# kazuto1011/dusty-gan

Measured on AMD Instinct MI355X. Metric: G+D train images/sec on 64x1024 LiDAR (steps/sec beside it), higher is better.
Workload: dtype bf16

## Files before the change

### dusty_gan_amd/_lib.py

```python
import ctypes as C
import os
import subprocess

_HERE = os.path.dirname(os.path.abspath(__file__))
CSRC = os.path.join(_HERE, "csrc")
LIB_PATH = os.path.join(CSRC, "libdustygan_hip.so")
if os.environ.get("DUSTY_GAN_LIB_DIAG"):
    _d = os.environ["DUSTY_GAN_LIB_DIAG"]
    LIB_PATH = os.path.join(CSRC, "libdustygan_hip_diag%s.so" % ("" if _d == "1" else _d))

DG_OK, DG_EINVAL, DG_EUNSUPPORTED, DG_EHIP = 0, 1, 2, 3
DG_F32, DG_BF16 = 0, 1
DG_BF16X2 = 2
MODE_S2, MODE_UP, MODE_GEMM = 0, 1, 2
EPI_LINEAR, EPI_LRELU, EPI_MASK = 0, 1, 2
DG_FORCE_AUTO, DG_FORCE_DIRECT, DG_FORCE_MFMA, DG_FORCE_THIN, DG_FORCE_LOCKSTEP, DG_FORCE_PINGPONG = 0, 1, 2, 3, 4, 5
DG_FORCE_WG_REGSTAGED, DG_FORCE_WG_DMA_PAIRS, DG_FORCE_WG_DMA_NOPAIRS, DG_FORCE_PINGPONG_SINGLE, DG_FORCE_PROJ_STREAM = 6, 7, 8, 9, 10
DG_FORCE_FP32X3 = 0x100
DG_CONV_FAMILY_DIRECT, DG_CONV_FAMILY_MFMA, DG_CONV_FAMILY_THIN, DG_CONV_FAMILY_LOCKSTEP, DG_CONV_FAMILY_PINGPONG = 1, 2, 3, 4, 5
DG_CONV_FAMILY_PROJ_STREAM = 6
DG_WGRAD_VARIANT_DIRECT, DG_WGRAD_VARIANT_MFMA, DG_WGRAD_VARIANT_THIN, DG_WGRAD_VARIANT_DMA, DG_WGRAD_VARIANT_THIN_MFMA = 1, 2, 3, 5, 7
POLICY_BITS = {"brightness": 1, "saturation": 2, "contrast": 4, "translation": 8, "cutout": 16}

_ERR = {1: "DG_EINVAL (bad argument)", 2: "DG_EUNSUPPORTED (shape not supported by the requested kernel)",
# ... 41 lines not shown
                ("eps", C.c_float), ("ilo", C.c_int), ("ihi", C.c_int), ("n", C.c_long), ("out", C.c_void_p),
                ("out_bf16", C.c_void_p), ("B", C.c_int), ("H", C.c_int), ("W", C.c_int), ("uf", C.c_void_p),
                ("qi", C.c_void_p)]


class DgWgrad(C.Structure):
    _fields_ = [
        ("wmode", C.c_int), ("ring", C.c_int),
        ("B", C.c_int), ("Hc", C.c_int), ("Wc", C.c_int),
        ("Ci", C.c_int), ("Co", C.c_int),
        ("a", C.c_void_p), ("a_sb", C.c_long), ("a_sp", C.c_long), ("a_sc", C.c_long),
        ("g", C.c_void_p), ("g_sb", C.c_long), ("g_sp", C.c_long), ("g_sc", C.c_long),
        ("dw", C.c_void_p), ("scale", C.c_float), ("rowscale", C.c_void_p),
        ("a_dtype", C.c_int), ("g_dtype", C.c_int),
        ("ws", C.c_void_p), ("g_mod", C.c_int),
    ]


XSUM_PARTS = 8


class DgFetch(C.Structure):
    _fields_ = [("pol", C.c_void_p), ("mask", C.c_void_p), ("pool_ctr", C.c_void_p), ("npool", C.c_int),
                ("min_depth", C.c_float), ("max_depth", C.c_float), ("drop_const", C.c_float), ("B", C.c_int), ("HW", C.c_long),
                ("out", C.c_void_p), ("parts", C.c_void_p), ("nslab", C.c_long), ("flip_tab", C.c_void_p)]


class DgAugSet(C.Structure):
    _fields_ = [("x", C.c_void_p), ("xsum", C.c_void_p), ("xsum_parts", C.c_int), ("u_b", C.c_void_p), ("u_c", C.c_void_p), ("t_h", C.c_void_p),
                ("t_w", C.c_void_p), ("o_x", C.c_void_p), ("o_y", C.c_void_p)]


class DgOptSeg(C.Structure):
    _fields_ = [("off", C.c_longlong), ("numel", C.c_longlong), ("part", C.c_void_p), ("splits", C.c_int), ("accumulate", C.c_int),
                ("kind", C.c_int), ("ci", C.c_int), ("co", C.c_int), ("shadow_t", C.c_void_p), ("ws_src", C.c_void_p),
                ("ws_coef", C.c_void_p), ("ws_stride", C.c_longlong), ("ws_n", C.c_int), ("ws_bf16", C.c_int),
                ("ws_scale", C.c_float), ("first_block", C.c_int)]


OPT_MAX_SEG = 20


class DgWgradPlan(C.Structure):
    _fields_ = [("variant", C.c_int), ("splits", C.c_int), ("ws_floats", C.c_long), ("tap_pairs", C.c_int)]


class DgWgradReduce(C.Structure):
    _fields_ = [("ws", C.c_void_p), ("dw", C.c_void_p), ("numel", C.c_long), ("splits", C.c_int), ("accumulate", C.c_int)]


class DgConvPlan(C.Structure):
    _fields_ = [("family", C.c_int), ("bm", C.c_int), ("bn", C.c_int), ("tiles", C.c_int), ("workgroups", C.c_int),
                ("tiles_per_wg", C.c_int), ("thin_mfma", C.c_int), ("mask_bits", C.c_int), ("dbias_rows", C.c_int),
                ("sum_parts", C.c_int)]


_P, _I, _L, _F, _D, _U64 = C.c_void_p, C.c_int, C.c_long, C.c_float, C.c_double, C.c_uint64

PROTOTYPES = {
    "dg_conv": [C.POINTER(DgConv), _I, _P],
    "dg_conv_ex": [C.POINTER(DgConv), _I, _I, _P],
    "dg_conv_plan": [C.POINTER(DgConv), _I, _I, C.POINTER(DgConvPlan)],
    "dg_conv_mfma_supported": [C.POINTER(DgConv)],
    "dg_wgrad": [C.POINTER(DgWgrad), _I, _I, _P],
    "dg_wgrad_plan": [C.POINTER(DgWgrad), _I, _I, C.POINTER(DgWgradPlan)],
    "dg_wgrad_group": [C.POINTER(DgWgrad), _I, _I, _I, _P],
    "dg_wgrad_group_plan": [C.POINTER(DgWgrad), _I, _I, _I, C.POINTER(DgWgradPlan)],
    "dg_wgrad_reduce": [C.POINTER(DgWgradReduce), _I, _P],
    "dg_wgrad_mfma_supported": [C.POINTER(DgWgrad)],
    "dg_wgrad_kernel_variant": [C.POINTER(DgWgrad), _I],
    "dg_wgrad_has_sample_map": [C.POINTER(DgWgrad), _I],
    "dg_blur_fwd": [_P, _P, _I, _I, _I, _I, _I, _P],
    "dg_blur_fwd_mean": [_P, _P, _I, _I, _I, _I, _I, _P, _I, _P, _P],
    "dg_blur_bwd": [_P, _I, _P, _I, _I, _I, _I, _P],
    "dg_blur_bwd_r1": [_P, _I, _P, _F, _P, _I, _I, _I, _I, _P],
    "dg_blur_r1_tangent": [_P, _I, _P, _F, _P, _P, _I, _I, _I, _I, _I, _P],
    "dg_final_fwd": [_P, _I, _P, _P, _F, _I, _L, _P, _P],
    "dg_final_fwd_acc": [_P, _I, _P, _P, _F, _I, _L, _P, _P],
    "dg_final_bwd_data": [_P, _I, _P, _P, _P, _F, _I, _L, _I, _P, _P, _P],
    "dg_batch_wsum": [_P, _I, _P, _F, _I, _L, _P, _P],
    "dg_head_post_fwd": [_P, _P, _P, _I, _I, _F, _F, _I, _L, _P, _P, _P],
    "dg_head_post_fwd_sum": [_P, _P, _P, _I, _I, _F, _F, _I, _L, _P, _P, _P, _P],
    "dg_head_post_bwd": [_P, _P, _P, _P, _P, _I, _F, _F, _I, _L, _F, _F, _P, _P, _P, _I, _P, _P],
    "dg_logistic_noise": [_P, _P, _F, _L, _P, _P],
    "dg_diffaug_fwd": [_P, _P, _P, _P, _P, _P, _P, _I, _I, _I, _I, _P, _P, _P],
    "dg_diffaug_bwd": [_P, _P, _P, _P, _P, _P, _P, _I, _I, _I, _I, _P, _P, _P],
    "dg_diffaug_fwd_acc": [_P, _P, _P, _P, _P, _P, _P, _I, _I, _I, _I, _P, _P, _P],
    "dg_diffaug_fwd_pre": [_P, _P, _P, _P, _P, _P, _P, _I, _I, _I, _I, _P, _P, _P],
    "dg_diffaug_bwd_acc": [_P, _P, _P, _P, _P, _P, _P, _I, _I, _I, _I, _P, _P, _P],
    "dg_diffaug_blur_fwd": [C.POINTER(DgAugSet), _I, _I, _I, _I, _I, _I, _P, _I, _P],
    "dg_blur_bwd_augsum": [_P, _I, _P, _P, _P, _P, _I, _P, _I, _I, _I, _I, _P],
    "dg_diffaug_bwd_pre": [_P, _P, _P, _P, _P, _P, _P, _I, _I, _I, _I, _P, _P, _P],
    "dg_head_post_bwd_aug": [_P, _P, _P, _P, _P, _P, _P, _P, _P, _P, _P, _I, _P, _I, _F, _F, _I, _I, _I, _F, _F, _P, _P, _P,
                             _I, _P, _P],
    "dg_fetch_reals_pool_sum": [_P, _P, _P, _I, _F, _F, _F, _I, _L, _P, _P, _P],
    "dg_fetch_reals_resident_sum": [_P, _P, _L, _P, _F, _F, _F, _I, _L, _P, _P, _P],
    "dg_resident_gather": [_P, _L, _I, _L, _L, _P, _P, _P, _P],
    "dg_nsgan_d": [_P, _P, _I, _F, _P, _P, _P, _P],
    "dg_nsgan_g": [_P, _I, _F, _P, _P, _P],
    "dg_nsgan_d_step": [_P, _P, _I, _F, _P, _P, _P, _P, _P, _P],
    "dg_nsgan_g_step": [_P, _I, _F, _P, _P, _P],
    "dg_gan_d_step": [_I, _F, _P, _P, _I, _F, _P, _P, _P, _P, _P, _P],
    "dg_gan_g_step": [_I, _P, _P, _I, _F, _P, _P, _P],
    "dg_final_gan_bwd": [_I, _I, _F, _P, _P, _I, _F, _I, _P, _P, _P, _P, _P, _P, _I, _P, _F, _L, _I, _P, _P, _P, _P, _P],
    "dg_det_arena": [_P, _L, _P],
    "dg_mean_acc": [_P, _I, _P, _P],
    "dg_fetch_reals": [_P, _P, _F, _F, _F, _L, _P, _P],
    "dg_fetch_reals_sum": [_P, _P, _F, _F, _F, _I, _L, _P, _P, _P],
    "dg_pl_penalty": [_P, _I, _I, _F, _P, _P, _P, _P],
    "dg_head_post_bwd2": [_P, _P, _P, _P, _P, _P, _I, _F, _F, _I, _L, _F, _F, _P, _P, _P, _I, _P],
    "dg_scan_to_polar": [_P, _I, _I, _I, _I, _I, _I, _P, _D, _D, _F, _P, _P, _P, _P, _P],
    "dg_inv_to_xyz": [_P, _P, _I, _I, _I, _I, _F, _F, _F, _F, _P, _P, _P],
    "dg_unit_map": [_P, _L, _I, _P, _P],
    "dg_normals": [_P, _I, _I, _I, _I, _P, _P],
    "dg_scan_project": [_P, _P, _I, _I, _I, _P, _P, _P, _P, _P],
# ... 328 lines not shown
```

### dusty_gan_amd/csrc/conv_mfma_persist_impl.h

```cpp
#pragma once
#include "mfma_common.h"

namespace persist {

template <typename T> struct StageWrite;
template <> struct StageWrite<bf16> {
  static __device__ __forceinline__ void put(unsigned addr, float v) {
    const bf16 h = (bf16)v;
    const unsigned bits = (unsigned)__builtin_bit_cast(unsigned short, h);
    asm volatile("ds_write_b16 %0, %1" ::"v"(addr), "v"(bits) : "memory");
  }
};
template <> struct StageWrite<float> {
  static __device__ __forceinline__ void put(unsigned addr, float v) {
    asm volatile("ds_write_b32 %0, %1" ::"v"(addr), "v"(v) : "memory");
  }
};

struct Tile {
  int nt, xt, px, Y, bt;
};

template <int MODE>
__device__ __forceinline__ bool next_tile(Tile& t, int tiles_n, int tiles_x, int rows) {
  if (++t.nt < tiles_n) return false;
  t.nt = 0;
  if (++t.xt < tiles_x) return false;
  t.xt = 0;
  if (MODE == MODE_UP) {
    if (++t.px < 2) return false;
    t.px = 0;
  }
  if (++t.Y == rows) { t.Y = 0; ++t.bt; }
  return true;
}

template <int MODE>
__host__ __device__ __forceinline__ int pack_htaps(int adj, int Y, int Hc, unsigned long long& list) {
  list = 0;
  int n = 0;
#pragma unroll
  for (int i = 0; i < 6; ++i) {
    int r, ky;
    if (dg_tap1d(MODE, adj, 0, Y, Hc, i, r, ky)) {
      list |= (unsigned long long)((r << 2) | ky) << (10 * n);
      ++n;
    }
  }
  return n;
}

#define DG_WAITV(n) asm volatile("s_waitcnt vmcnt(%0)" ::"n"(n) : "memory")

struct Geo {
  int tiles_n, tiles_x, ntiles;
  int SW, NSB, lsw;
  int dbg;
};

template <typename T, int BM, int BN, int WM, int WN, int SB, int NS, int MODE>
__global__ __launch_bounds__(64 * WM * WN, 1) void conv_kernel(ConvP p, Geo g) {
  constexpr int NWV = WM * WN;
  constexpr int ES = sizeof(T);
  constexpr int BK = SB / ES;
  constexpr int EPC = 16 / ES;
  constexpr int TM = BM / WM / 32, TN = BN / WN / 32;
  constexpr int RPI = 1024 / SB;
  constexpr int CPR = SB / 16;
  constexpr int KS = SB / 32;
  constexpr int STAGE = (BM + BN) * SB;
  constexpr int IA = BM / RPI / NWV, IB = BN / RPI / NWV;
  constexpr int IPT = IA + IB;
  constexpr int E = NS - 1;
  constexpr int WC = BN / WN;
  constexpr int RB = WC * ES;
  constexpr int RS = RB + 16;
  constexpr int CR = RB / 16;
  constexpr int NDB0 = 512;
  constexpr int DBR = sizeof(T) == 4 ? WM : 1;
  constexpr int SR = (NS * STAGE + NWV * 16 * RS + NDB0 * 4 * DBR > 160 * 1024) ? 8 : 16;
  constexpr int CPL = SR * CR / 64;
  constexpr int STRIP = SR * RS;
  constexpr int NQ = 32 / SR;
  constexpr int NST = TM * NQ * CPL;
  constexpr int nW = MODE == MODE_S2 ? 4 : 2;
  static_assert(IA >= 1 && IB >= 1, "piece distribution");
  static_assert(NS >= 3 && NS <= 4 && KS >= 2 && KS % 2 == 0 && 2 * IPT + NST <= 63, "ring / vmcnt immediates");
  constexpr int NDB = 512;
  static_assert(NS * STAGE + NWV * STRIP + NDB * 4 * DBR <= 160 * 1024, "LDS");
  __shared__ __attribute__((aligned(1024))) unsigned char lds[NS * STAGE + NWV * STRIP + NDB * 4 * DBR];

  const int G = gridDim.x;
  const int q8 = G >> 3, r8 = G & 7, xcd = blockIdx.x & 7;
  const int gi = (xcd < r8 ? xcd * (q8 + 1) : r8 * (q8 + 1) + (xcd - r8) * q8) + (blockIdx.x >> 3);
  const int tq = g.ntiles / G, tr = g.ntiles % G;
  const int t0 = gi * tq + (gi < tr ? gi : tr);
  const int tcount = tq + (gi < tr ? 1 : 0);
  if (tcount == 0) return;

  const int tid = threadIdx.x;
  const int KC = p.K / BK;
  const int Ws = MODE == MODE_S2 ? 2 * p.Wc : p.Wc, cmul = MODE == MODE_S2 ? 2 : 1;
  const int Wo = MODE == MODE_S2 ? p.Wc : 2 * p.Wc;
  const int rows = MODE == MODE_S2 ? p.Hc : 2 * p.Hc;
  const int tiles_n = g.tiles_n, tiles_x = g.tiles_x;

  Tile first;
  {
    int mt = t0 / tiles_n;
    first.nt = t0 % tiles_n;
// ... 386 lines not shown
```

### dusty_gan_amd/csrc/conv_mfma_pp.hip

```cpp
#include "conv_mfma_persist_impl.h"

#include <type_traits>

namespace pp {

using persist::Geo;
using persist::Tile;

typedef __attribute__((ext_vector_type(4))) float f32x4_t;

#define PP_WAIT(vm) asm volatile("s_waitcnt vmcnt(%0) lgkmcnt(0)" ::"n"(vm) : "memory")

constexpr int NHT = 256;
struct HTab { unsigned long long e[NHT]; };

__device__ __forceinline__ unsigned long long pp_stamp() {
  unsigned long long t;
  __builtin_amdgcn_sched_barrier(0);
  asm volatile("s_memtime %0\n\ts_waitcnt lgkmcnt(0)" : "=s"(t)::"memory");
  __builtin_amdgcn_sched_barrier(0);
  return t;
}

template <int CTRL>
__device__ __forceinline__ float row_add(float v) {
  const int s = __builtin_amdgcn_update_dpp(0, __builtin_bit_cast(int, v), CTRL, 0xf, 0xf, false);
  return v + __builtin_bit_cast(float, s);
}

template <int BN, int MODE, bool MASK, bool DUAL = false, bool BITS = false, bool X2 = false>
__global__ __launch_bounds__(512, 2) void conv_pp_kernel(ConvP p, Geo g, HTab ht) {
  static_assert(MASK || !BITS, "BITS: a flavour of the EPI_MASK epilogue");
  static_assert(!X2 || !BITS, "X2: mask source = the saved activation's hi half");
  static_assert(!DUAL || (MODE == MODE_UP && BN == 128), "DUAL: both column parities of a 64-channel MODE_UP layer");
  constexpr int NCH = DUAL ? BN / 2 : BN;
  constexpr int BM = 256, NWV = 8, WN = 2;
  constexpr int SB = 128;
  constexpr int WC = BN / WN;
  constexpr int TM = 4, TN = WC / 16;
  constexpr int CPL = 4 * TN;
  constexpr int IMG_ROWS = 264;
  constexpr int AIMG = IMG_ROWS * SB;
  constexpr int BT = BN * SB;
  constexpr int PSTAGE = AIMG + 2 * BT;
  constexpr int NPS = 2;
  constexpr int IA = 4, IB = BN / 8 / NWV;
  constexpr int NST = TM * CPL * 2 / 16;
  constexpr int NDB = 512;
  constexpr int NPAIR = MODE == MODE_S2 ? 2 : 1;
  constexpr bool STRIP = BN == 128 && !X2;
  constexpr int SCR = STRIP ? 16 * WC * 2 : 0;
  constexpr int NDBR = 4;
  constexpr int NDBX = MASK ? (NDBR - 2) * NDB : 0;
  constexpr int DBW = DUAL ? NWV : NWV / WN;
  constexpr int LDS_HT = NPS * PSTAGE + 3 * NDB * 4 + NDBX * 4 + NWV * SCR;
  static_assert(IB >= 1 && LDS_HT <= 160 * 1024, "LDS");
  __shared__ __attribute__((aligned(1024))) unsigned char lds[LDS_HT];
#ifdef DG_PP_DIAG
  constexpr int dbg = DG_PP_DIAG;
#else
  constexpr int dbg = 0;
#endif

  const int G = gridDim.x;
  const int q8 = G >> 3, r8 = G & 7, xcd = blockIdx.x & 7;
  const int gi0 = xcd < r8 ? xcd * (q8 + 1) : r8 * (q8 + 1) + (xcd - r8) * q8;
  const int nwx = q8 + (xcd < r8 ? 1 : 0);
  const int tq = g.ntiles / G, tr = g.ntiles % G;
  const int xs = gi0 * tq + (gi0 < tr ? gi0 : tr);
  const int xe = (gi0 + nwx) * tq + (gi0 + nwx < tr ? gi0 + nwx : tr);
  const int t0 = xs + (int)(blockIdx.x >> 3);
  const int tcount = t0 < xe ? (xe - t0 + nwx - 1) / nwx : 0;
  if (tcount == 0) {
    if (MASK && p.dbias && p.dbias_part)
      for (int n = threadIdx.x; n < p.N; n += 64 * NWV) p.dbias_part[(long)blockIdx.x * p.N + n] = 0.f;
    return;
  }

  const unsigned long long tk0 = (dbg & 8) ? pp_stamp() : 0ull;
  const unsigned long long tr0 = (dbg & 8) ? __builtin_amdgcn_s_memrealtime() : 0ull;
  const int tid = threadIdx.x;
  const int wave = __builtin_amdgcn_readfirstlane(tid >> 6), lane = tid & 63;
  const int KC = p.K / 64;
  const int Ws = MODE == MODE_S2 ? 2 * p.Wc : p.Wc, cmul = MODE == MODE_S2 ? 2 : 1;
  const int Wo = MODE == MODE_S2 ? p.Wc : 2 * p.Wc;
  const int rows = MODE == MODE_S2 ? p.Hc : 2 * p.Hc;
  const int tiles_n = g.tiles_n, tiles_x = g.tiles_x;

  auto tile_at = [&](int t) {
    Tile r;
    int mt = t / tiles_n;
    r.nt = t % tiles_n;
    r.px = 0;
    r.xt = mt % tiles_x; mt /= tiles_x;
    if (MODE == MODE_UP && !DUAL) { r.px = mt & 1; mt >>= 1; }
    r.Y = mt % rows; r.bt = mt / rows;
    r.nt = __builtin_amdgcn_readfirstlane(r.nt); r.xt = __builtin_amdgcn_readfirstlane(r.xt);
    r.px = __builtin_amdgcn_readfirstlane(r.px); r.Y = __builtin_amdgcn_readfirstlane(r.Y);
    r.bt = __builtin_amdgcn_readfirstlane(r.bt);
    return r;
  };
  const Tile first = tile_at(t0);
  Tile dstep;
  {
    int r = nwx;
    dstep.nt = r % tiles_n; r /= tiles_n;
    dstep.xt = r % tiles_x; r /= tiles_x;
    dstep.px = 0;
    if (MODE == MODE_UP && !DUAL) { dstep.px = r & 1; r >>= 1; }
    dstep.Y = r % rows; dstep.bt = r / rows;
    dstep.nt = __builtin_amdgcn_readfirstlane(dstep.nt); dstep.xt = __builtin_amdgcn_readfirstlane(dstep.xt);
    dstep.px = __builtin_amdgcn_readfirstlane(dstep.px); dstep.Y = __builtin_amdgcn_readfirstlane(dstep.Y);
    dstep.bt = __builtin_amdgcn_readfirstlane(dstep.bt);
  }
  auto tile_next = [&](Tile& t) __attribute__((always_inline)) {
    int c;
    t.nt += dstep.nt; c = t.nt >= tiles_n; if (c) t.nt -= tiles_n;
    t.xt += dstep.xt + c; c = t.xt >= tiles_x; if (c) t.xt -= tiles_x;
    if (MODE == MODE_UP && !DUAL) { t.px += dstep.px + c; c = t.px >> 1; t.px &= 1; }
    t.Y += dstep.Y + c; c = t.Y >= rows; if (c) t.Y -= rows;
    t.bt += dstep.bt + c;
  };

  const bf16* in = (const bf16*)p.in;
  const bf16* w = (const bf16*)p.w;
  const int lrow = lane >> 3, pos = lane & 7;
  auto swzA = [](int row) { return ((row >> 1) & 3) << 1; };
  auto swzB = [](int row) { return ((row >> 1) & 1) | (((row / CPL) & 3) << 1); };

  unsigned voffA[NPAIR][IA + 1], voffB[IB];
  int colA[IA + 1];
  unsigned sampA[IA + 1];
  {
    const int pitch = g.SW + (DUAL ? 2 : 1);
#pragma unroll
    for (int u = 0; u <= IA; ++u) {
      const int m = (u < IA ? (wave + NWV * u) : 32) * 8 + lrow;
      int seg = m / pitch, c = m - seg * pitch;
      if (seg >= g.NSB) { seg = 0; c = 0; }
      colA[u] = cmul * c;
      sampA[u] = (unsigned)(seg * (int)p.in_sb * 2 + (pos ^ swzA(m)) * 16);
    }
  }
#pragma unroll
  for (int u = 0; u < IB; ++u) {
    const int row = (wave + NWV * u) * 8 + lrow;
    voffB[u] = (unsigned)((DUAL ? row & 63 : row) * (int)p.w_sn * 2 + (pos ^ swzB(row)) * 16);
  }
  const unsigned dst_wave = (unsigned)wave * 1024u;

  const int wm = wave >> 1, wn = wave & 1;
  const int a16 = lane & 15, g4 = lane >> 4;
  const unsigned lds0 = (unsigned)(size_t)(__attribute__((address_space(3))) unsigned char*)lds;
  unsigned pbase[2];
  {
    const int rowbase = ((wm * 64) >> g.lsw) * (g.SW + (DUAL ? 2 : 1)) + ((wm * 64) & (g.SW - 1));
#pragma unroll
    for (int t = 0; t < 2; ++t) {
      const int r = rowbase + a16 + t + (DUAL ? wn : 0);
      pbase[t] = (unsigned)(r * SB + ((g4 ^ swzA(r)) << 4));
    }
  }
  const unsigned wrow = (unsigned)(wn * WC + (a16 >> 2) * CPL + (a16 & 3));
  const unsigned wbase = (unsigned)(AIMG + wrow * SB + ((g4 ^ (((a16 >> 1) & 1) | ((a16 >> 2) << 1))) << 4));

  float* s_rs = (float*)(lds + NPS * PSTAGE);
  float* s_bias = s_rs + NDB;
  float* s_db = s_bias + NDB;
  const unsigned srs0 = lds0 + NPS * PSTAGE, sbias0 = srs0 + NDB * 4, sdb0 = sbias0 + NDB * 4;
  const bool want_db = MASK && p.dbias != nullptr;
  const bool db_rows = MASK && DBW * p.N <= NDBR * NDB;
  const unsigned sdbw0 = db_rows ? sbias0 + (unsigned)((DUAL ? wave : wave / WN) * p.N) * 4u : sdb0;
  for (int i = tid; i < NDB; i += 64 * NWV) {
    s_bias[i] = (!MASK && p.bias && i < p.N) ? p.bias[i % p.bias_mod] * (p.epi == EPI_LRELU ? SQRT2 : 1.f) : 0.f;
    s_db[i] = 0.f;
// ... 281 lines not shown
      else if (t == 0) { if (wave == 0) PP_WAIT(IA + IB + 1); else PP_WAIT(IA + IB); }
      else PP_WAIT(IB);
      auto finish_tile = [&]() __attribute__((always_inline)) {
        if (!(dbg & 4)) epilogue(tprev);
        else {
#pragma unroll
          for (int i = 0; i < TM; ++i)
#pragma unroll
            for (int jj = 0; jj < TN; ++jj) asm volatile("" ::"v"(acc[i][jj]));
          zero_acc();
        }
        pending = false;
      };
      if (t == 0 && pending && wave >= 4) finish_tile();
      if (stamps) t2 = pp_stamp();
      __builtin_amdgcn_s_barrier();
      if (stamps) t3 = pp_stamp();
      __builtin_amdgcn_sched_barrier(0);
      if (t == 0 && pending) finish_tile();
      __builtin_amdgcn_sched_barrier(0);
      if (comp) {
        if (stamps && tkf == 0) tkf = t3;
#pragma unroll
        for (int ks = 0; ks < 2; ++ks) {
          if (!(dbg & 2)) {
#pragma unroll
            for (int i = 0; i < TM; ++i)
#pragma unroll
              for (int jj = 0; jj < TN; ++jj)
                acc[i][jj] = __builtin_amdgcn_mfma_f32_16x16x32_bf16(__builtin_bit_cast(bf16x8, fw[ks][jj]),
                                                                      __builtin_bit_cast(bf16x8, fp[ks][i]), acc[i][jj], 0, 0, 0);
          }
          if (ks == 0) {
            __builtin_amdgcn_sched_barrier(0);
            if (MASK && last && !(dbg & (4 | 64))) load_aux(tprev);
          }
        }
        if (last) pending = true;
      }
      __builtin_amdgcn_sched_barrier(0);
      if (stamps) t4 = pp_stamp();
      if (ISS || t == 0 || wave < 4) __builtin_amdgcn_s_barrier();
      if (stamps) {
        t5 = pp_stamp();
        tsum[0] += t1 - t0; tsum[1] += t2 - t1; tsum[2] += t3 - t2; tsum[3] += t4 - t3; tsum[4] += t5 - t4;
        tend = t5;
      }
    };
    step(std::integral_constant<int, 0>{});
    step(std::integral_constant<int, 1>{});
    const unsigned sw_ = so_c; so_c = so_i; so_i = sw_;
  };

  Tile ti = first;
  for (int c = 0; c < tcount; ++c) {
    unsigned long long hl;
    int nh;
    {
      const unsigned long long e = ht.e[ti.Y];
      nh = (int)(e >> 60) & 7;
      hl = e & 0x0fffffffffffffffull;
    }
    const char* in_t = (const char*)(in + (long)(ti.bt * g.NSB) * p.in_sb);
    const char* w_t = (const char*)(w + (long)(ti.nt * NCH) * p.w_sn);
    const int x0 = cmul * ti.xt * BM;
#pragma unroll
    for (int pi = 0; pi < NPAIR; ++pi) {
      const int cb = MODE == MODE_S2 ? pi - 1 : ((DUAL || ti.px == 0) ? -1 : 0);
#pragma unroll
      for (int u = 0; u <= IA; ++u)
        voffA[pi][u] = __umul24((unsigned)((x0 + colA[u] + cb) & (Ws - 1)), spb) + sampA[u];
    }
    const int kxa = MODE == MODE_S2 ? 0 : (ti.px == 0 ? 3 : 2), kxb = MODE == MODE_S2 ? 2 : (ti.px == 0 ? 1 : 0);
    bool firstg = true;
    for (int h = 0; h < nh; ++h) {
      const int it_r = (int)(hl & 1023) >> 2, it_ky = (int)hl & 3;
      hl >>= 10;
      const char* sA_row = in_t + (long)it_r * Ws * spb;
      const char* sB_row = w_t + (long)(it_ky * 4) * tap_b;
      for (int kc = 0; kc < (X2 ? 3 : 1) * KC; ++kc) {
        const int kq = X2 ? kc / 3 : kc, sub = X2 ? kc - 3 * kq : 0;
        const char* sA_k = sA_row + kq * (X2 ? 2 * SB : SB) + (sub == 1 ? SB : 0);
        const char* sB_k = sB_row + kq * (X2 ? 2 * SB : SB) + (sub == 2 ? SB : 0);
#pragma unroll
        for (int pi = 0; pi < NPAIR; ++pi) {
          pair_iter(std::true_type{}, firstg, pi, sA_k, sB_k + (long)(kxa + pi) * tap_b, sB_k + (long)(kxb + pi) * tap_b,
                    sB_k + 2 * tap_b, sB_k);
          if (firstg) { firstg = false; warm = false; }
        }
      }
    }
    tprev = ti;
    tile_next(ti);
  }
  pair_iter(std::false_type{}, true, 0, nullptr, nullptr, nullptr, nullptr, nullptr);
  const unsigned long long tk2 = (dbg & 8) ? pp_stamp() : 0ull;
  const unsigned long long tr2 = (dbg & 8) ? __builtin_amdgcn_s_memrealtime() : 0ull;
  if (pending && !(dbg & 4)) {
    asm volatile("s_waitcnt vmcnt(0)" ::: "memory");
    epilogue(tprev);
  }
  if (stamps && blockIdx.x == 0 && lane == 0) {
    float* sink = (float*)p.out + wave * 8;
    asm volatile("s_waitcnt vmcnt(0)" ::: "memory");
    const unsigned long long tk3 = pp_stamp();
    for (int k = 0; k < 6; ++k) sink[k] = (float)tsum[k];
    float* ph = (float*)p.out + 64 + wave * 8;
    ph[0] = (float)(tk1 - tk0); ph[1] = (float)(tkf - tk0); ph[2] = (float)(tk2 - tk0); ph[3] = (float)(tk3 - tk0);
    ph[4] = (float)tcount;
    ph[5] = (float)(tr2 - tr0);
  }
  if (want_db) {
    asm volatile("s_waitcnt vmcnt(0) lgkmcnt(0)" ::: "memory");
    __syncthreads();
    for (int n = tid; n < p.N; n += 64 * NWV) {
      float v;
      if (db_rows) {
        v = s_bias[n];
#pragma unroll
        for (int r = 1; r < DBW; ++r) v += s_bias[r * p.N + n];
      } else v = s_db[n];
      if (p.dbias_part) p.dbias_part[(long)blockIdx.x * p.N + n] = v;
      else atomicAdd(&p.dbias[n % p.bias_mod], v);
    }
  }
}

template <int BN, int MODE, bool MASK, bool DUAL = false, bool X2 = false>
int launch(const ConvP* p, const Geo& g0, hipStream_t stream, int wg_cap, DgConvPlan* plan) {
  constexpr int CPL_ = (BN / 2 / 16) * 4;
  const bool bits_ok = !X2 && p->out_sn == 1 && p->out_sb % 8 == 0 && p->out_sp % CPL_ == 0 && p->N % CPL_ == 0;
  if (!MASK && p->mask_out && !bits_ok) return DG_EUNSUPPORTED;
  const bool bits = MASK && p->mask_in && bits_ok;
  Geo g = g0;
  static int resident = 0;
  if (!resident) {
    int dev = 0, cus = 0;
    HIP_CHECK_RET(hipGetDevice(&dev));
    HIP_CHECK_RET(hipDeviceGetAttribute(&cus, hipDeviceAttributeMultiprocessorCount, dev));
    resident = cus;
  }
  g.dbg = 0;
  const int cap = (wg_cap > 0 && wg_cap < resident) ? wg_cap : resident;
  const int G = g.ntiles < cap ? g.ntiles : cap;
  if (plan) {
    plan->family = DG_CONV_FAMILY_PINGPONG; plan->bm = DUAL ? 512 : 256; plan->bn = DUAL ? BN / 2 : BN; plan->tiles = g.ntiles; plan->workgroups = G;
    plan->tiles_per_wg = (g.ntiles + G - 1) / G;
    plan->mask_bits = MASK ? (bits ? 2 : 0) : 1;
    plan->dbias_rows = (MASK && (DUAL ? 8 : 4) * p->N <= 2048) ? G : 0;
    return DG_OK;
  }
  HTab ht;
  {
    const int rows = MODE == MODE_S2 ? p->Hc : 2 * p->Hc;
    for (int y = 0; y < NHT; ++y) {
      unsigned long long hl = 0;
      const int nh = y < rows ? persist::pack_htaps<MODE>(p->adj, y, p->Hc, hl) : 0;
      ht.e[y] = hl | ((unsigned long long)nh << 60);
    }
  }
  if constexpr (X2) {
    conv_pp_kernel<BN, MODE, MASK, DUAL, false, true><<<(unsigned)G, 512, 0, stream>>>(*p, g, ht);
  } else if constexpr (MASK) {
    if (bits) conv_pp_kernel<BN, MODE, true, DUAL, true><<<(unsigned)G, 512, 0, stream>>>(*p, g, ht);
    else conv_pp_kernel<BN, MODE, true, DUAL, false><<<(unsigned)G, 512, 0, stream>>>(*p, g, ht);
  } else conv_pp_kernel<BN, MODE, false, DUAL><<<(unsigned)G, 512, 0, stream>>>(*p, g, ht);
  HIP_CHECK_RET(hipGetLastError());
  return DG_OK;
}

}

int dg_conv_mfma_pp_launch(const ConvP* p0, hipStream_t stream, int min_tiles, int wg_cap, DgConvPlan* plan, int dual) {
  if (p0->mode != MODE_S2 && p0->mode != MODE_UP) return DG_EUNSUPPORTED;
  const bool x2 = p0->in_dtype == DG_BF16X2;
  if (p0->in_dtype != p0->out_dtype || p0->in_dtype != p0->w_dtype || (p0->in_dtype != DG_BF16 && !x2)) return DG_EUNSUPPORTED;
  ConvP q = *p0;
  if (x2) {
    if (p0->K % 64 || p0->N % 64 || p0->in_sp % 64 || p0->in_sb % 64 || p0->out_sp % 64 || p0->out_sb % 64 || p0->w_sn % 64 ||
        p0->w_st % 64 || (((size_t)p0->in | (size_t)p0->out | (size_t)p0->w | (size_t)p0->aux) & 255))
      return DG_EUNSUPPORTED;
    if (p0->mask_out || p0->mask_in) return DG_EUNSUPPORTED;
    q.in_sb *= 2; q.in_sp *= 2; q.out_sb *= 2; q.out_sp *= 2; q.w_st *= 2; q.w_sn *= 2;
  }
  const ConvP* p = &q;
  if (p->K % 64 != 0 || !p->ring || p->nscale) return DG_EUNSUPPORTED;
  if (p->mode == MODE_UP && p->adj && p->K < 128) return DG_EUNSUPPORTED;
  if (p->in_sk != 1 || p->w_sk != 1 || p->out_sn != 1) return DG_EUNSUPPORTED;
  if (p->out_sp % 8 != 0 || p->in_sp % 8 != 0 || p->w_sn % 8 != 0) return DG_EUNSUPPORTED;
  if (p->N > 512 || (p->bias && p->bias_mod < p->N && p->N % p->bias_mod != 0)) return DG_EUNSUPPORTED;
  if (p->dbias && p->bias_mod < p->N) return DG_EUNSUPPORTED;
  const int Ws = p->mode == MODE_S2 ? 2 * p->Wc : p->Wc;
  if ((Ws & (Ws - 1)) != 0 || p->in_sp * 2 >= (1 << 24)) return DG_EUNSUPPORTED;
  if ((p->mode == MODE_S2 ? p->Hc : 2 * p->Hc) > 256) return DG_EUNSUPPORTED;
  const bool mask = p->epi == EPI_MASK;
  if (mask ? p->bias != nullptr : p->dbias != nullptr) return DG_EUNSUPPORTED;
  if (p->rowscale && p->B > 512) return DG_EUNSUPPORTED;
  persist::Geo g;
  int bn = 0;
  if (dual && p->mode == MODE_UP && p->N % 128 != 0 && p->N % 64 == 0 && persist::make_geo<256, 64>(p, g) && g.SW >= 64 &&
      g.NSB * (g.SW + 2) <= 264 && g.ntiles / 2 >= min_tiles) {
    g.ntiles /= 2;
    if (x2) return mask ? pp::launch<128, MODE_UP, true, true, true>(p, g, stream, wg_cap, plan)
                        : pp::launch<128, MODE_UP, false, true, true>(p, g, stream, wg_cap, plan);
    return mask ? pp::launch<128, MODE_UP, true, true>(p, g, stream, wg_cap, plan)
                : pp::launch<128, MODE_UP, false, true>(p, g, stream, wg_cap, plan);
  }
  if (p->N % 128 == 0 && persist::make_geo<256, 128>(p, g) && g.SW >= 64 && g.ntiles >= min_tiles) bn = 128;
  else if (p->N % 64 == 0 && persist::make_geo<256, 64>(p, g) && g.SW >= 64 && g.ntiles >= min_tiles) bn = 64;
  if (!bn) return DG_EUNSUPPORTED;
  const int sel = (bn == 128 ? 0 : 4) + (p->mode == MODE_UP ? 2 : 0) + (mask ? 1 : 0);
  if (x2) switch (sel) {
    case 0: return pp::launch<128, MODE_S2, false, false, true>(p, g, stream, wg_cap, plan);
    case 1: return pp::launch<128, MODE_S2, true, false, true>(p, g, stream, wg_cap, plan);
    case 2: return pp::launch<128, MODE_UP, false, false, true>(p, g, stream, wg_cap, plan);
    case 3: return pp::launch<128, MODE_UP, true, false, true>(p, g, stream, wg_cap, plan);
    case 4: return pp::launch<64, MODE_S2, false, false, true>(p, g, stream, wg_cap, plan);
    case 5: return pp::launch<64, MODE_S2, true, false, true>(p, g, stream, wg_cap, plan);
    case 6: return pp::launch<64, MODE_UP, false, false, true>(p, g, stream, wg_cap, plan);
    default: return pp::launch<64, MODE_UP, true, false, true>(p, g, stream, wg_cap, plan);
  }
  switch (sel) {
    case 0: return pp::launch<128, MODE_S2, false>(p, g, stream, wg_cap, plan);
// ... 10 lines not shown
```

### include/dusty_gan_hip.h

```cpp
#ifndef DUSTY_GAN_HIP_H
#define DUSTY_GAN_HIP_H
#include <stdint.h>

#ifdef __cplusplus
extern "C" {
#endif

#define DG_OK 0
#define DG_EINVAL 1
#define DG_EUNSUPPORTED 2
#define DG_EHIP 3

#define DG_F32 0
#define DG_BF16 1
#define DG_BF16X2 2

#define DG_MODE_S2 0
#define DG_MODE_UP 1
#define DG_MODE_GEMM 2

#define DG_EPI_LINEAR 0
#define DG_EPI_LRELU 1
#define DG_EPI_MASK 2

// ... 22 lines not shown
  void* mask_out;
  const void* mask_in;
  float* tanh_sum_parts;
} DgConv;
#define DG_UP_FRAG_BYTES (3 * 18 * 1024)
#define DG_DBIAS_SLOTS 32
#define DG_DBIAS_SLOT_FLOATS 1024

typedef struct DgWgrad {
  int wmode, ring;
  int B, Hc, Wc;
  int Ci, Co;
  const void* a;
  long a_sb, a_sp, a_sc;
  const void* g;
  long g_sb, g_sp, g_sc;
  float* dw;
  float scale;
  const float* rowscale;
  int a_dtype, g_dtype;
  float* ws;
  int g_mod;
} DgWgrad;

int dg_conv(const DgConv* p, int force, void* stream);
#define DG_FORCE_AUTO 0
#define DG_FORCE_DIRECT 1
#define DG_FORCE_MFMA 2
#define DG_FORCE_THIN 3
#define DG_FORCE_LOCKSTEP 4
#define DG_FORCE_PINGPONG 5
#define DG_FORCE_WG_REGSTAGED 6
#define DG_FORCE_WG_DMA_PAIRS 7
#define DG_FORCE_WG_DMA_NOPAIRS 8
#define DG_FORCE_PINGPONG_SINGLE 9
#define DG_FORCE_PROJ_STREAM 10
#define DG_FORCE_FP32X3 0x100
#define DG_CONV_FAMILY_DIRECT 1
#define DG_CONV_FAMILY_MFMA 2
#define DG_CONV_FAMILY_THIN 3
#define DG_CONV_FAMILY_LOCKSTEP 4
#define DG_CONV_FAMILY_PINGPONG 5
#define DG_CONV_FAMILY_PROJ_STREAM 6
typedef struct DgConvPlan {
  int family;
  int bm, bn;
  int tiles;
  int workgroups;
  int tiles_per_wg;
  int thin_mfma;
  int mask_bits;
  int dbias_rows;
  int sum_parts;
} DgConvPlan;
int dg_conv_ex(const DgConv* p, int force, int wg_cap, void* stream);
int dg_conv_plan(const DgConv* p, int force, int wg_cap, DgConvPlan* plan);
int dg_conv_mfma_supported(const DgConv* p);

int dg_wgrad(const DgWgrad* p, int accumulate, int force, void* stream);
#define DG_WGRAD_VARIANT_DIRECT 1
#define DG_WGRAD_VARIANT_MFMA 2
#define DG_WGRAD_VARIANT_THIN 3
#define DG_WGRAD_VARIANT_DMA 5
#define DG_WGRAD_VARIANT_THIN_MFMA 7
typedef struct DgWgradPlan {
  int variant;
  int splits;
  long ws_floats;
  int tap_pairs;
} DgWgradPlan;
int dg_wgrad_plan(const DgWgrad* p, int accumulate, int force, DgWgradPlan* plan);
int dg_wgrad_group(const DgWgrad* items, int n, int force, int rounds, void* stream);
int dg_wgrad_group_plan(const DgWgrad* items, int n, int force, int rounds, DgWgradPlan* plans);
typedef struct DgWgradReduce {
  const float* ws;
  float* dw;
  long numel;
  int splits;
  int accumulate;
} DgWgradReduce;
int dg_wgrad_reduce(const DgWgradReduce* items, int n, void* stream);
int dg_wgrad_mfma_supported(const DgWgrad* p);
int dg_wgrad_kernel_variant(const DgWgrad* p, int force);
int dg_wgrad_has_sample_map(const DgWgrad* p, int force);

int dg_blur_fwd(const float* x, void* out, int dtype, int B, int H, int W, int ring, void* stream);
int dg_blur_fwd_mean(const float* x, void* out, int dtype, int B, int H, int W, int ring, const float* mean_src, int mean_n,
                     float* mean_acc, void* stream);
int dg_blur_bwd(const void* d, int dtype, float* dx, int B, int H, int W, int ring, void* stream);
int dg_blur_bwd_r1(const void* d, int dtype, float* dx, float oscale, float* ssq, int B, int H, int W, int ring, void* stream);
int dg_blur_r1_tangent(const void* d, int dtype, void* out, float oscale, float* ssq, float* mean_acc, int mean_n, int B, int H,
                       int W, int ring, void* stream);

int dg_final_fwd(const void* d4, int dtype, const float* wf, const float* bias, float scale, int B, long n, float* y,
                 void* stream);
int dg_final_fwd_acc(const void* d4, int dtype, const float* wf, const float* bias, float scale, int B, long n, float* y,
                 void* stream);
int dg_final_bwd_data(const void* d4, int dtype, const float* wf, const float* up, const float* rowscale, float scale,
                      int B, long n, int C, void* dd4, float* dbias, void* stream);
int dg_batch_wsum(const void* src, int dtype, const float* coef, float scale, int B, long n, float* out, void* stream);

int dg_head_post_fwd(float* gout, const float* noise_pixel, const float* noise_image, int arch, int training,
                     float tau, float drop_const, int B, long HW, float* mask, float* depth, void* stream);
int dg_head_post_fwd_sum(float* gout, const float* noise_pixel, const float* noise_image, int arch, int training,
                         float tau, float drop_const, int B, long HW, float* mask, float* depth, float* dsum, void* stream);
int dg_head_post_bwd(const float* gout, const float* noise_pixel, const float* noise_image, const float* mask,
                     const float* ddepth, int arch, float tau, float drop_const, int B, long HW, float s_depth,
                     float s_conf, float* draw, float* dbias, void* draw_pm , int cp,
                     float* bias_ws, void* stream);
// ... 209 lines not shown
```

Before: 14020.

## Rotate ping-pong conv tile walk to balance per-workgroup tap load

Replaces the fixed strided tile walk in the persistent ping-pong conv kernel with a parameterised walk. Each workgroup's stride can advance by one extra row of tiles per step, which spreads rows with different vertical-tap counts more evenly across workgroups. The host simulates per-workgroup tap work for both walks and picks the rotated one only when it lowers the maximum. The choice is cached per shape, and the old walk is kept for masked dbias kernels or when an env var requests it. It adds host-side simulation cost on cache misses and a slightly more complex device-side tile increment.

```diff
diff --git a/dusty_gan_amd/_lib.py b/dusty_gan_amd/_lib.py
--- a/dusty_gan_amd/_lib.py
+++ b/dusty_gan_amd/_lib.py
@@ -117,7 +117,10 @@
 class DgConvPlan(C.Structure):
     _fields_ = [("family", C.c_int), ("bm", C.c_int), ("bn", C.c_int), ("tiles", C.c_int), ("workgroups", C.c_int),
                 ("tiles_per_wg", C.c_int), ("thin_mfma", C.c_int), ("mask_bits", C.c_int), ("dbias_rows", C.c_int),
-                ("sum_parts", C.c_int)]
+                ("sum_parts", C.c_int),
+                ("tiles_n", C.c_int), ("tiles_x", C.c_int), ("tile_par", C.c_int), ("tile_rows", C.c_int),
+                ("walk_shift", C.c_int), ("walk_units", C.c_long), ("walk_max_units", C.c_int),
+                ("walk_max_units_old", C.c_int)]
 
 
 _P, _I, _L, _F, _D, _U64 = C.c_void_p, C.c_int, C.c_long, C.c_float, C.c_double, C.c_uint64
@@ -126,6 +129,7 @@
     "dg_conv": [C.POINTER(DgConv), _I, _P],
     "dg_conv_ex": [C.POINTER(DgConv), _I, _I, _P],
     "dg_conv_plan": [C.POINTER(DgConv), _I, _I, C.POINTER(DgConvPlan)],
+    "dg_conv_walk_order": [C.POINTER(DgConvPlan), _I, C.POINTER(C.c_int), _L],
     "dg_conv_mfma_supported": [C.POINTER(DgConv)],
     "dg_wgrad": [C.POINTER(DgWgrad), _I, _I, _P],
     "dg_wgrad_plan": [C.POINTER(DgWgrad), _I, _I, C.POINTER(DgWgradPlan)],
diff --git a/dusty_gan_amd/csrc/conv_mfma_persist_impl.h b/dusty_gan_amd/csrc/conv_mfma_persist_impl.h
--- a/dusty_gan_amd/csrc/conv_mfma_persist_impl.h
+++ b/dusty_gan_amd/csrc/conv_mfma_persist_impl.h
@@ -56,6 +56,7 @@
   int tiles_n, tiles_x, ntiles;
   int SW, NSB, lsw;
   int dbg;
+  int shift = 0;
 };
 
 template <typename T, int BM, int BN, int WM, int WN, int SB, int NS, int MODE>
diff --git a/dusty_gan_amd/csrc/conv_mfma_pp.hip b/dusty_gan_amd/csrc/conv_mfma_pp.hip
--- a/dusty_gan_amd/csrc/conv_mfma_pp.hip
+++ b/dusty_gan_amd/csrc/conv_mfma_pp.hip
@@ -1,5 +1,7 @@
 #include "conv_mfma_persist_impl.h"
 
+#include <cstdlib>
+#include <cstring>
 #include <type_traits>
 
 namespace pp {
@@ -8,6 +10,62 @@
 using persist::Tile;
 
 typedef __attribute__((ext_vector_type(4))) float f32x4_t;
+
+__host__ __device__ __forceinline__ int walk_uni(int v) {
+#if defined(__HIP_DEVICE_COMPILE__)
+  return __builtin_amdgcn_readfirstlane(v);
+#else
+  return v;
+#endif
+}
+
+template <bool PAR>
+struct Walk {
+  Tile t;
+  int count;
+  Tile dn, dw;
+  int pos, nwx, shift, tiles_n, tiles_x, rows;
+
+  __host__ __device__ __forceinline__ Tile digits(int r) const {
+    Tile d;
+    d.nt = r % tiles_n; r /= tiles_n;
+    d.xt = r % tiles_x; r /= tiles_x;
+    d.px = 0;
+    if (PAR) { d.px = r & 1; r >>= 1; }
+    d.Y = r % rows; d.bt = r / rows;
+    d.nt = walk_uni(d.nt); d.xt = walk_uni(d.xt); d.px = walk_uni(d.px); d.Y = walk_uni(d.Y); d.bt = walk_uni(d.bt);
+    return d;
+  }
+  __host__ __device__ __forceinline__ void init(int G, int block, int ntiles, int tiles_n_, int tiles_x_, int rows_, int shift_) {
+    tiles_n = tiles_n_; tiles_x = tiles_x_; rows = rows_; shift = shift_;
+    const int q8 = G >> 3, r8 = G & 7, xcd = block & 7;
+    const int gi0 = xcd < r8 ? xcd * (q8 + 1) : r8 * (q8 + 1) + (xcd - r8) * q8;
+    nwx = q8 + (xcd < r8 ? 1 : 0);
+    const int tq = ntiles / G, tr = ntiles % G;
+    const int xs = gi0 * tq + (gi0 < tr ? gi0 : tr);
+    const int xe = (gi0 + nwx) * tq + (gi0 + nwx < tr ? gi0 + nwx : tr);
+    pos = block >> 3;
+    const int nfull = (xe - xs) / nwx, rem = (xe - xs) - nfull * nwx;
+    count = nfull + ((pos + nfull * shift) % nwx < rem ? 1 : 0);
+    t = digits(xs + pos);
+    dn = digits(nwx + shift);
+    dw = digits(shift);
+  }
+  __host__ __device__ __forceinline__ void next() {
+    pos += shift;
+    const bool wrap = pos >= nwx;
+    if (wrap) pos -= nwx;
+    int c;
+    t.nt += wrap ? dw.nt : dn.nt; c = t.nt >= tiles_n; if (c) t.nt -= tiles_n;
+    t.xt += (wrap ? dw.xt : dn.xt) + c; c = t.xt >= tiles_x; if (c) t.xt -= tiles_x;
+    if (PAR) { t.px += (wrap ? dw.px : dn.px) + c; c = t.px >> 1; t.px &= 1; }
+    t.Y += (wrap ? dw.Y : dn.Y) + c; c = t.Y >= rows; if (c) t.Y -= rows;
+    t.bt += (wrap ? dw.bt : dn.bt) + c;
+  }
+  __host__ __device__ __forceinline__ int linear() const {
+    return (((t.bt * rows + t.Y) * (PAR ? 2 : 1) + t.px) * tiles_x + t.xt) * tiles_n + t.nt;
+  }
+};
 
 #define PP_WAIT(vm) asm volatile("s_waitcnt vmcnt(%0) lgkmcnt(0)" ::"n"(vm) : "memory")
 
@@ -62,15 +120,10 @@
   constexpr int dbg = 0;
 #endif
 
-  const int G = gridDim.x;
-  const int q8 = G >> 3, r8 = G & 7, xcd = blockIdx.x & 7;
-  const int gi0 = xcd < r8 ? xcd * (q8 + 1) : r8 * (q8 + 1) + (xcd - r8) * q8;
-  const int nwx = q8 + (xcd < r8 ? 1 : 0);
-  const int tq = g.ntiles / G, tr = g.ntiles % G;
-  const int xs = gi0 * tq + (gi0 < tr ? gi0 : tr);
-  const int xe = (gi0 + nwx) * tq + (gi0 + nwx < tr ? gi0 + nwx : tr);
-  const int t0 = xs + (int)(blockIdx.x >> 3);
-  const int tcount = t0 < xe ? (xe - t0 + nwx - 1) / nwx : 0;
+  constexpr bool PAR = MODE == MODE_UP && !DUAL;
+  Walk<PAR> walk;
+  walk.init((int)gridDim.x, (int)blockIdx.x, g.ntiles, g.tiles_n, g.tiles_x, MODE == MODE_S2 ? p.Hc : 2 * p.Hc, g.shift);
+  const int tcount = walk.count;
   if (tcount == 0) {
     if (MASK && p.dbias && p.dbias_part)
       for (int n = threadIdx.x; n < p.N; n += 64 * NWV) p.dbias_part[(long)blockIdx.x * p.N + n] = 0.f;
@@ -84,43 +137,7 @@
   const int KC = p.K / 64;
   const int Ws = MODE == MODE_S2 ? 2 * p.Wc : p.Wc, cmul = MODE == MODE_S2 ? 2 : 1;
   const int Wo = MODE == MODE_S2 ? p.Wc : 2 * p.Wc;
-  const int rows = MODE == MODE_S2 ? p.Hc : 2 * p.Hc;
-  const int tiles_n = g.tiles_n, tiles_x = g.tiles_x;
-
-  auto tile_at = [&](int t) {
-    Tile r;
-    int mt = t / tiles_n;
-    r.nt = t % tiles_n;
-    r.px = 0;
-    r.xt = mt % tiles_x; mt /= tiles_x;
-    if (MODE == MODE_UP && !DUAL) { r.px = mt & 1; mt >>= 1; }
-    r.Y = mt % rows; r.bt = mt / rows;
-    r.nt = __builtin_amdgcn_readfirstlane(r.nt); r.xt = __builtin_amdgcn_readfirstlane(r.xt);
-    r.px = __builtin_amdgcn_readfirstlane(r.px); r.Y = __builtin_amdgcn_readfirstlane(r.Y);
-    r.bt = __builtin_amdgcn_readfirstlane(r.bt);
-    return r;
-  };
-  const Tile first = tile_at(t0);
-  Tile dstep;
-  {
-    int r = nwx;
-    dstep.nt = r % tiles_n; r /= tiles_n;
-    dstep.xt = r % tiles_x; r /= tiles_x;
-    dstep.px = 0;
-    if (MODE == MODE_UP && !DUAL) { dstep.px = r & 1; r >>= 1; }
-    dstep.Y = r % rows; dstep.bt = r / rows;
-    dstep.nt = __builtin_amdgcn_readfirstlane(dstep.nt); dstep.xt = __builtin_amdgcn_readfirstlane(dstep.xt);
-    dstep.px = __builtin_amdgcn_readfirstlane(dstep.px); dstep.Y = __builtin_amdgcn_readfirstlane(dstep.Y);
-    dstep.bt = __builtin_amdgcn_readfirstlane(dstep.bt);
-  }
-  auto tile_next = [&](Tile& t) __attribute__((always_inline)) {
-    int c;
-    t.nt += dstep.nt; c = t.nt >= tiles_n; if (c) t.nt -= tiles_n;
-    t.xt += dstep.xt + c; c = t.xt >= tiles_x; if (c) t.xt -= tiles_x;
-    if (MODE == MODE_UP && !DUAL) { t.px += dstep.px + c; c = t.px >> 1; t.px &= 1; }
-    t.Y += dstep.Y + c; c = t.Y >= rows; if (c) t.Y -= rows;
-    t.bt += dstep.bt + c;
-  };
+  const Tile first = walk.t;
 
   const bf16* in = (const bf16*)p.in;
   const bf16* w = (const bf16*)p.w;
@@ -508,8 +525,8 @@
     const unsigned sw_ = so_c; so_c = so_i; so_i = sw_;
   };
 
-  Tile ti = first;
   for (int c = 0; c < tcount; ++c) {
+    const Tile ti = walk.t;
     unsigned long long hl;
     int nh;
     {
@@ -547,7 +564,7 @@
       }
     }
     tprev = ti;
-    tile_next(ti);
+    walk.next();
   }
   pair_iter(std::false_type{}, true, 0, nullptr, nullptr, nullptr, nullptr, nullptr);
   const unsigned long long tk2 = (dbg & 8) ? pp_stamp() : 0ull;
@@ -582,6 +599,59 @@
   }
 }
 
+struct WalkCost { long total; int max_units; };
+template <bool PAR>
+WalkCost walk_cost(int G, const Geo& g, int rows, const int* nh, int shift, int* order, int per_wg) {
+  WalkCost c{0, 0};
+  for (int b = 0; b < G; ++b) {
+    Walk<PAR> w;
+    w.init(G, b, g.ntiles, g.tiles_n, g.tiles_x, rows, shift);
+    int sum = 0;
+    for (int i = 0; i < w.count; ++i, w.next()) {
+      sum += nh[w.t.Y];
+      if (order && i < per_wg) order[(long)b * per_wg + i] = w.linear();
+    }
+    c.total += sum;
+    if (sum > c.max_units) c.max_units = sum;
+  }
+  return c;
+}
+inline WalkCost walk_cost(bool par, int G, const Geo& g, int rows, const int* nh, int shift, int* order = nullptr, int per_wg = 0) {
+  return par ? walk_cost<true>(G, g, rows, nh, shift, order, per_wg) : walk_cost<false>(G, g, rows, nh, shift, order, per_wg);
+}
+
+struct WalkPick { int shift; long total; int max_units, max_old; };
+inline WalkPick pick_shift(bool par, int G, const Geo& g, int rows, const int* nh) {
+  struct Key { int par, G, ntiles, tiles_n, tiles_x, rows; unsigned long long sig; };
+  struct Ent { Key k; WalkPick v; };
+  thread_local Ent cache[8];
+  thread_local int used = 0, victim = 0;
+  unsigned long long sig = 1469598103934665603ull;
+  bool uniform = true;
+  for (int y = 0; y < rows; ++y) { sig = (sig ^ (unsigned)nh[y]) * 1099511628211ull; uniform = uniform && nh[y] == nh[0]; }
+  const Key k{par ? 1 : 0, G, g.ntiles, g.tiles_n, g.tiles_x, rows, sig};
+  for (int i = 0; i < used; ++i) {
+    const Key& c = cache[i].k;
+    if (c.par == k.par && c.G == k.G && c.ntiles == k.ntiles && c.tiles_n == k.tiles_n && c.tiles_x == k.tiles_x &&
+        c.rows == k.rows && c.sig == k.sig) return cache[i].v;
+  }
+  const WalkCost old = walk_cost(par, G, g, rows, nh, 0);
+  WalkPick v{0, old.total, old.max_units, old.max_units};
+  const int row_tiles = g.tiles_n * g.tiles_x * (par ? 2 : 1);
+  if (!uniform && row_tiles < (G >> 3) && g.ntiles >= 2 * G) {
+    const WalkCost rot = walk_cost(par, G, g, rows, nh, row_tiles);
+    if (rot.max_units < old.max_units) { v.shift = row_tiles; v.max_units = rot.max_units; }
+  }
+  const int slot = used < 8 ? used++ : (victim = (victim + 1) & 7);
+  cache[slot] = Ent{k, v};
+  return v;
+}
+
+inline bool walk_forced_old() {
+  const char* e = getenv("DUSTY_GAN_PP_WALK");
+  return e && !strcmp(e, "old");
+}
+
 template <int BN, int MODE, bool MASK, bool DUAL = false, bool X2 = false>
 int launch(const ConvP* p, const Geo& g0, hipStream_t stream, int wg_cap, DgConvPlan* plan) {
   constexpr int CPL_ = (BN / 2 / 16) * 4;
@@ -590,30 +660,39 @@
   const bool bits = MASK && p->mask_in && bits_ok;
   Geo g = g0;
   static int resident = 0;
-  if (!resident) {
+  const bool assumed = plan && wg_cap < 0;
+  if (!resident && !assumed) {
     int dev = 0, cus = 0;
     HIP_CHECK_RET(hipGetDevice(&dev));
     HIP_CHECK_RET(hipDeviceGetAttribute(&cus, hipDeviceAttributeMultiprocessorCount, dev));
     resident = cus;
   }
   g.dbg = 0;
-  const int cap = (wg_cap > 0 && wg_cap < resident) ? wg_cap : resident;
+  const int cap = assumed ? -wg_cap : ((wg_cap > 0 && wg_cap < resident) ? wg_cap : resident);
   const int G = g.ntiles < cap ? g.ntiles : cap;
+  constexpr bool PAR = MODE == MODE_UP && !DUAL;
+  const int rows = MODE == MODE_S2 ? p->Hc : 2 * p->Hc;
+  HTab ht;
+  int nhs[NHT];
+  for (int y = 0; y < NHT; ++y) {
+    unsigned long long hl = 0;
+    const int nh = y < rows ? persist::pack_htaps<MODE>(p->adj, y, p->Hc, hl) : 0;
+    ht.e[y] = hl | ((unsigned long long)nh << 60);
+    nhs[y] = nh;
+  }
+  const WalkPick pick = pick_shift(PAR, G, g, rows, nhs);
+  g.shift = (walk_forced_old() || (MASK && p->dbias)) ? 0 : pick.shift;
   if (plan) {
     plan->family = DG_CONV_FAMILY_PINGPONG; plan->bm = DUAL ? 512 : 256; plan->bn = DUAL ? BN / 2 : BN; plan->tiles = g.ntiles; plan->workgroups = G;
     plan->tiles_per_wg = (g.ntiles + G - 1) / G;
     plan->mask_bits = MASK ? (bits ? 2 : 0) : 1;
     plan->dbias_rows = (MASK && (DUAL ? 8 : 4) * p->N <= 2048) ? G : 0;
+    plan->tiles_n = g.tiles_n; plan->tiles_x = g.tiles_x; plan->tile_par = PAR ? 2 : 1; plan->tile_rows = rows;
+    plan->walk_shift = g.shift;
+    plan->walk_units = pick.total;
+    plan->walk_max_units = g.shift ? pick.max_units : pick.max_old;
+    plan->walk_max_units_old = pick.max_old;
     return DG_OK;
-  }
-  HTab ht;
-  {
-    const int rows = MODE == MODE_S2 ? p->Hc : 2 * p->Hc;
-    for (int y = 0; y < NHT; ++y) {
-      unsigned long long hl = 0;
-      const int nh = y < rows ? persist::pack_htaps<MODE>(p->adj, y, p->Hc, hl) : 0;
-      ht.e[y] = hl | ((unsigned long long)nh << 60);
-    }
   }
   if constexpr (X2) {
     conv_pp_kernel<BN, MODE, MASK, DUAL, false, true><<<(unsigned)G, 512, 0, stream>>>(*p, g, ht);
@@ -625,6 +704,19 @@
   return DG_OK;
 }
 
+}
+
+extern "C" int dg_conv_walk_order(const DgConvPlan* plan, int shift, int* order, long n) {
+  if (!plan || !order || plan->family != DG_CONV_FAMILY_PINGPONG || plan->workgroups < 1 || plan->tiles < plan->workgroups)
+    return DG_EINVAL;
+  if (shift < 0 || (shift > 0 && shift >= plan->workgroups >> 3)) return DG_EINVAL;
+  if (n < (long)plan->workgroups * plan->tiles_per_wg) return DG_EINVAL;
+  for (long i = 0; i < n; ++i) order[i] = -1;
+  pp::Geo g{};
+  g.ntiles = plan->tiles; g.tiles_n = plan->tiles_n; g.tiles_x = plan->tiles_x;
+  int nh[pp::NHT] = {};
+  pp::walk_cost(plan->tile_par == 2, plan->workgroups, g, plan->tile_rows, nh, shift, order, plan->tiles_per_wg);
+  return DG_OK;
 }
 
 int dg_conv_mfma_pp_launch(const ConvP* p0, hipStream_t stream, int min_tiles, int wg_cap, DgConvPlan* plan, int dual) {
diff --git a/include/dusty_gan_hip.h b/include/dusty_gan_hip.h
--- a/include/dusty_gan_hip.h
+++ b/include/dusty_gan_hip.h
@@ -98,9 +98,16 @@
   int mask_bits;
   int dbias_rows;
   int sum_parts;
+  int tiles_n, tiles_x;
+  int tile_par, tile_rows;
+  int walk_shift;
+  long walk_units;
+  int walk_max_units;
+  int walk_max_units_old;
 } DgConvPlan;
 int dg_conv_ex(const DgConv* p, int force, int wg_cap, void* stream);
 int dg_conv_plan(const DgConv* p, int force, int wg_cap, DgConvPlan* plan);
+int dg_conv_walk_order(const DgConvPlan* plan, int shift, int* order, long n);
 int dg_conv_mfma_supported(const DgConv* p);
 
 int dg_wgrad(const DgWgrad* p, int accumulate, int force, void* stream);
```

After: 13770. 1.8% lower.
